# Smaug123/ray-tracing-fsharp

Measured on AMD Instinct MI355X. Metric: Mray/s (primary+secondary), higher is better.
Workload: dtype f64

## Files before the change

ray-tracing-fsharp_amd/csrc/rt_device.h:

```cpp
#pragma once
#include "rt_launch_consts.h"
#include <hip/hip_runtime.h>
#include <stdint.h>
#include <type_traits>

#include "rt_trig.h"

#pragma clang fp contract(off)

namespace rtd {

#define RTD_INLINE __device__ __forceinline__
#define RTD_AS3 __attribute__((address_space(3)))

typedef double d2 __attribute__((ext_vector_type(2)));
typedef int i2 __attribute__((ext_vector_type(2)));
typedef int i4 __attribute__((ext_vector_type(4)));

#define RTD_TOL 0.00000001
RTD_INLINE bool feq(double a, double b) { return fabs(a - b) < RTD_TOL; }
RTD_INLINE bool fpos(double a) { return a > RTD_TOL; }
enum { CMP_GT = 0, CMP_EQ = 1, CMP_LT = 2 };
RTD_INLINE int fcmp(double a, double b) {
    if (fabs(a - b) < RTD_TOL) return CMP_EQ;
// ... 16 lines not shown
    g = fma(g, r, g);
    h = fma(h, r, h);
    double e = fma(-g, g, x);
    g = fma(e, h, g);
    e = fma(-g, g, x);
    return fma(e, h, g);
}
RTD_INLINE double rcp_core(double s) {
    double r = __builtin_amdgcn_rcp(s);
    double e = fma(-s, r, 1.0);
    r = fma(r, e, r);
    e = fma(-s, r, 1.0);
    r = fma(r, e, r);
    e = fma(-s, r, 1.0);
    return fma(e, r, r);
}
RTD_INLINE double sqrt_above_tol(double x) {
    const double g = sqrt_core(x);
    return __builtin_isinf(x) ? x : g;
}
RTD_INLINE double inv_sqrt_above_tol(double x) {
    const double q = rcp_core(sqrt_core(x));
    return __builtin_isinf(x) ? 0.0 : q;
}
RTD_INLINE bool unitise(V3 v, V3 &out) {
    double d = dot(v, v);
    if (feq(d, 0.0)) return false;
    double factor = inv_sqrt_above_tol(d);
    out = vscale(factor, v);
    return true;
}

#ifdef RTD_STAGE_CLOCKS
#define RTD_CENSUS_WORDS 48
__device__ unsigned long long g_census[RTD_CENSUS_WORDS];
#define RTD_CENSUS_EVENT(i) atomicAdd(&g_census[i], 1ull)
#else
#define RTD_CENSUS_EVENT(i)
#endif

struct Rng { uint32_t x, y, z, w; };
RTD_INLINE uint32_t rng_next(Rng &r) {
    uint32_t t = r.x ^ (r.x << 11);
    r.x = r.y;
    r.y = r.z;
    r.z = r.w;
    r.w = r.w ^ (r.w >> 19) ^ (t ^ (t >> 8));
    return r.w;
}
RTD_INLINE double rng_get(Rng &r) {
    const double x = (double) __builtin_bswap32(rng_next(r));
    return fma(x, 0x1p-64 + 0x1p-96, x * 0x1p-32);
}

__host__ __device__ __forceinline__ uint64_t mix64(uint64_t z) {
    z ^= z >> 30;
    z *= 0xBF58476D1CE4E5B9ull;
    z ^= z >> 27;
    z *= 0x94D049BB133111EBull;
    z ^= z >> 31;
    return z;
}
#define RTD_GOLDEN 0x9E3779B97F4A7C15ull
RTD_INLINE uint32_t mod_m31(uint32_t x) {
    const uint32_t r = (x & 0x7FFFFFFFu) + (x >> 31);
    return r >= 2147483647u ? r - 2147483647u : r;
}
// ... 227 lines not shown
        "  v_min_f64 v[102:103], v[106:107], v[102:103]\n"
        "  s_waitcnt lgkmcnt(1)\n"
        "  v_add_f64 v[108:109], v[108:109], -%[oz]\n"
        "  v_mul_f64 v[108:109], %[iz], v[108:109]\n"
        "  v_max_f64 v[100:101], v[108:109], v[100:101]\n"
        "  v_add_f64 v[110:111], v[110:111], -%[oz]\n"
        "  v_mul_f64 v[110:111], %[iz], v[110:111]\n"
        "  v_cmp_lt_f64 vcc, 0, v[102:103]\n"
        "  v_min_f64 v[102:103], v[110:111], v[102:103]\n"
        "  v_cmp_ge_f64 %[save2], v[102:103], v[100:101]\n"
        "  s_and_b64 vcc, vcc, %[save2]\n"
        "  s_waitcnt lgkmcnt(0)\n"
        "  v_cndmask_b32 %[off], v113, v112, vcc\n"
        "  v_cndmask_b32 v113, 0, v115, vcc\n"
        "  v_alignbit_b32 %[pend], v114, %[pend], v113\n"
        "  s_mov_b64 exec, %[save]\n"
        "  s_branch 1b\n"
        "2:\n"
        : [off] "+v"(off), [pend] "+v"(pend), [ax] "=&v"(ax), [ay] "=&v"(ay), [az] "=&v"(az), [cnt] "=&s"(cnt), [save] "=&s"(save), [save2] "=&s"(save2)
        : [end] "s"(end), [stop] "s"(stop), [nx] "v"(c.nX), [ny] "v"(c.nY), [nz] "v"(c.nZ), [ox] "v"(o.x), [oy] "v"(o.y), [oz] "v"(o.z),
          [ix] "v"(c.ix), [iy] "v"(c.iy), [iz] "v"(c.iz), [inf] "s"(inf)
        : "vcc", "scc", "memory", "v100", "v101", "v102", "v103", "v104", "v105", "v106", "v107", "v108", "v109", "v110", "v111", "v112", "v113",
          "v114", "v115");
    return off;
}
#define RTD_PEND_MARK 0x4000u

struct WalkCtx32 {
    float ix, iy, iz;
    float cnx, cny, cnz;
    float cfx, cfy, cfz;
    int nX, nY, nZ;
};
RTD_INLINE void filter_axis(double o, double d, float bmax, float &inv, float &cn, float &cf, int &nOff) {
    inv = __builtin_amdgcn_rcpf((float) d);
    const float oi = (float) o * inv;
    const float m = fmaf(__builtin_fabsf(inv), bmax, __builtin_fabsf(oi)) * 0x1p-20f + 1e-30f;
    cn = -oi - m;
    cf = m - oi;
    nOff = (int) (((uint32_t) __double2hiint(d) >> 28) & 8u);
}
RTD_INLINE WalkCtx32 walk_ctx32(V3 o, V3 d, float bmax) {
    WalkCtx32 c;
    filter_axis(o.x, d.x, bmax, c.ix, c.cnx, c.cfx, c.nX);
    filter_axis(o.y, d.y, bmax, c.iy, c.cny, c.cfy, c.nY);
    filter_axis(o.z, d.z, bmax, c.iz, c.cnz, c.cfz, c.nZ);
    return c;
}
RTD_INLINE bool bbox_filter(const WalkCtx32 &c, float lox, float hix, float loy, float hiy, float loz, float hiz) {
    const float tn = __builtin_fmaxf(__builtin_fmaxf(__builtin_fmaxf(fmaf(c.nX ? hix : lox, c.ix, c.cnx), fmaf(c.nY ? hiy : loy, c.iy, c.cny)),
                                                     fmaf(c.nZ ? hiz : loz, c.iz, c.cnz)), 0.0f);
    const float tf = __builtin_fminf(__builtin_fminf(fmaf(c.nX ? lox : hix, c.ix, c.cfx), fmaf(c.nY ? loy : hiy, c.iy, c.cfy)), fmaf(c.nZ ? loz : hiz, c.iz, c.cfz));
    return !(tf < tn);
}
#ifdef RTD_STAGE_CLOCKS
#define RTD_TRIP_COUNT(S) S
#define RTD_TRIP_ARGS , unsigned &trips, unsigned &lanes
#define RTD_TRIP_OPS , [trips] "+s"(trips), [lanes] "+s"(lanes)
#else
#define RTD_TRIP_COUNT(S)
#define RTD_TRIP_ARGS
#define RTD_TRIP_OPS
#endif
RTD_INLINE int node_loop_lds32(int off, uint32_t &pend, int end, int stop, const WalkCtx32 &c RTD_TRIP_ARGS) {
    int ax, ay, az, cnt;
    unsigned long long save, save2;
#ifdef RTD_PK_FMA
    auto pk = [](float lo, float hi) { return ((unsigned long long) __float_as_uint(hi) << 32) | (unsigned long long) __float_as_uint(lo); };
    const unsigned long long pix = pk(c.ix, c.ix), piy = pk(c.iy, c.iy), piz = pk(c.iz, c.iz);
    const unsigned long long pcx = pk(c.cnx, c.cfx), pcy = pk(c.cny, c.cfy), pcz = pk(c.cnz, c.cfz);
#endif
    asm volatile(
        "s_waitcnt lgkmcnt(0)\n"
        "1:\n"
        "  v_cmp_gt_i32 vcc, %[end], %[off]\n"
        "  v_cmp_eq_u16 %[save2], 0, %[pend]\n"
        "  s_and_b64 vcc, vcc, %[save2]\n"
        "  s_bcnt1_i32_b64 %[cnt], vcc\n"
        "  s_cmp_le_u32 %[cnt], %[stop]\n"
        "  s_cbranch_scc1 2f\n"
        "  s_and_saveexec_b64 %[save], vcc\n"
        RTD_TRIP_COUNT("  s_add_u32 %[trips], %[trips], 1\n  s_add_u32 %[lanes], %[lanes], %[cnt]\n")
        "  v_add_u32 %[ax], %[off], %[nx]\n"
        "  v_add_u32 %[ay], %[off], %[ny]\n"
        "  v_add_u32 %[az], %[off], %[nz]\n"
        "  ds_read_b64 v[100:101], %[ax]\n"
        "  ds_read_b64 v[102:103], %[ay] offset:16\n"
        "  ds_read_b64 v[104:105], %[az] offset:32\n"
        "  ds_read_b128 v[106:109], %[off] offset:48\n"
        "  s_waitcnt lgkmcnt(3)\n"
#ifdef RTD_PK_FMA
        "  v_pk_fma_f32 v[100:101], v[100:101], %[pix], %[pcx] op_sel_hi:[1,0,1]\n"
        "  s_waitcnt lgkmcnt(2)\n"
        "  v_pk_fma_f32 v[102:103], v[102:103], %[piy], %[pcy] op_sel_hi:[1,0,1]\n"
        "  s_waitcnt lgkmcnt(1)\n"
        "  v_pk_fma_f32 v[104:105], v[104:105], %[piz], %[pcz] op_sel_hi:[1,0,1]\n"
#else
        "  v_fma_f32 v100, v100, %[ix], %[cnx]\n"
        "  v_fma_f32 v101, v101, %[ix], %[cfx]\n"
        "  s_waitcnt lgkmcnt(2)\n"
        "  v_fma_f32 v102, v102, %[iy], %[cny]\n"
        "  v_fma_f32 v103, v103, %[iy], %[cfy]\n"
        "  s_waitcnt lgkmcnt(1)\n"
        "  v_fma_f32 v104, v104, %[iz], %[cnz]\n"
        "  v_fma_f32 v105, v105, %[iz], %[cfz]\n"
#endif
        "  v_max3_f32 v100, v100, v102, v104\n"
        "  v_min3_f32 v101, v101, v103, v105\n"
        "  v_max_f32 v100, 0, v100\n"
        "  v_cmp_nlt_f32 vcc, v101, v100\n"
        "  s_waitcnt lgkmcnt(0)\n"
        "  v_cndmask_b32 %[off], v107, v106, vcc\n"
        "  v_cndmask_b32 v107, 0, v109, vcc\n"
        "  v_alignbit_b32 %[pend], v108, %[pend], v107\n"
        "  s_mov_b64 exec, %[save]\n"
        "  s_branch 1b\n"
        "2:\n"
        : [off] "+v"(off), [pend] "+v"(pend), [ax] "=&v"(ax), [ay] "=&v"(ay), [az] "=&v"(az), [cnt] "=&s"(cnt), [save] "=&s"(save), [save2] "=&s"(save2) RTD_TRIP_OPS
        : [end] "s"(end), [stop] "s"(stop), [nx] "v"(c.nX), [ny] "v"(c.nY), [nz] "v"(c.nZ), [ix] "v"(c.ix), [iy] "v"(c.iy), [iz] "v"(c.iz),
          [cnx] "v"(c.cnx), [cny] "v"(c.cny), [cnz] "v"(c.cnz), [cfx] "v"(c.cfx), [cfy] "v"(c.cfy), [cfz] "v"(c.cfz)
#ifdef RTD_PK_FMA
          , [pix] "v"(pix), [piy] "v"(piy), [piz] "v"(piz), [pcx] "v"(pcx), [pcy] "v"(pcy), [pcz] "v"(pcz)
#endif
        : "vcc", "scc", "memory", "v100", "v101", "v102", "v103", "v104", "v105", "v106", "v107", "v108", "v109");
    return off;
}
RTD_INLINE int pend_pop(uint32_t &pend) {
    const uint32_t lo = pend & 0xFFFFu;
    const uint32_t e = lo != 0u ? lo : (pend >> 16);
    pend = lo != 0u ? (pend & 0xFFFF0000u) : 0u;
    return (int) (e & (RTD_PEND_MARK - 1u));
}
template <bool LDS>
RTD_INLINE void leaf_test(const SceneView<LDS> &sc, V3 o, V3 d, WalkCtx &c, Walk &w) {
    typedef typename Ptrs<LDS>::bp bp;
    bp rec = node_at<LDS>(sc, w.off & (RTD_LEAF - 1));
    const int next = *(typename Ptrs<LDS>::ip) (rec + 100), prim = *(typename Ptrs<LDS>::ip) (rec + 104);
    const d2 g0 = sc.geo[prim * 3 + 0], g1 = sc.geo[prim * 3 + 1];
    const double t = sphere_first_intersection(o, d, mk(g0.x, g0.y, g1.x), g1.y);
    const double a = t * t;
    if (a < c.bestF || (a == c.bestF && prim < w.best)) { c.bestF = a; w.best = prim; w.bestLen = t; }
    w.off = next;
// ... 16 lines not shown
        "  v_cmp_eq_u32 %[save2], 0, %[pend1]\n"
        "  s_and_b64 vcc, vcc, %[save2]\n"
        "  s_bcnt1_i32_b64 %[cnt], vcc\n"
        "  s_cmp_le_u32 %[cnt], %[stop]\n"
        "  s_cbranch_scc1 2f\n"
        "  s_and_saveexec_b64 %[save], vcc\n"
        "  v_add_u32 %[ax], %[off], %[nx]\n"
        "  v_add_u32 %[ay], %[off], %[ny]\n"
        "  v_add_u32 %[az], %[off], %[nz]\n"
        "  v_cmp_gt_i32 vcc, %[lim], %[off]\n"
        "  s_bcnt1_i32_b64 %[cnt], vcc\n"
        "  s_cmp_ge_u32 %[cnt], %[thr]\n"
        "  s_cbranch_scc1 3f\n"
        "  s_and_saveexec_b64 %[save2], vcc\n"
        "  ds_read_b64 v[100:101], %[ax]\n"
        "  ds_read_b64 v[102:103], %[ay] offset:16\n"
        "  ds_read_b64 v[104:105], %[az] offset:32\n"
        "  ds_read_b128 v[106:109], %[off] offset:48\n"
        "  s_andn2_b64 exec, %[save2], exec\n"
        "  global_load_dwordx2 v[100:101], %[ax], %[base]\n"
        "  global_load_dwordx2 v[102:103], %[ay], %[base] offset:16\n"
        "  global_load_dwordx2 v[104:105], %[az], %[base] offset:32\n"
        "  global_load_dwordx4 v[106:109], %[off], %[base] offset:48\n"
        "  s_mov_b64 exec, %[save2]\n"
        "  s_branch 4f\n"
        "3:\n"
        "  s_mov_b64 exec, vcc\n"
        "  ds_read_b64 v[100:101], %[ax]\n"
        "  ds_read_b64 v[102:103], %[ay] offset:16\n"
        "  ds_read_b64 v[104:105], %[az] offset:32\n"
        "  ds_read_b128 v[106:109], %[off] offset:48\n"
        "4:\n"
        "  s_waitcnt vmcnt(0) lgkmcnt(0)\n"
        "  v_fma_f32 v100, v100, %[ix], %[cnx]\n"
        "  v_fma_f32 v101, v101, %[ix], %[cfx]\n"
        "  v_fma_f32 v102, v102, %[iy], %[cny]\n"
        "  v_fma_f32 v103, v103, %[iy], %[cfy]\n"
        "  v_fma_f32 v104, v104, %[iz], %[cnz]\n"
        "  v_fma_f32 v105, v105, %[iz], %[cfz]\n"
        "  v_max3_f32 v100, v100, v102, v104\n"
        "  v_min3_f32 v101, v101, v103, v105\n"
        "  v_max_f32 v100, 0, v100\n"
        "  v_cmp_nlt_f32 vcc, v101, v100\n"
        "  v_cndmask_b32 %[off], v107, v106, vcc\n"
        "  v_cndmask_b32 v108, 0, v108, vcc\n"
        "  v_cmp_ne_u32 %[save3], 0, v108\n"
        "  v_cmp_eq_u32 vcc, 0, %[pend0]\n"
        "  s_and_b64 vcc, %[save3], vcc\n"
        "  v_cndmask_b32 %[pend0], %[pend0], v108, vcc\n"
        "  s_andn2_b64 vcc, %[save3], vcc\n"
        "  v_cndmask_b32 %[pend1], %[pend1], v108, vcc\n"
        "  s_mov_b64 exec, %[save]\n"
        "  s_branch 1b\n"
        "2:\n"
        : [off] "+v"(off), [pend0] "+v"(pend0), [pend1] "+v"(pend1), [ax] "=&v"(ax), [ay] "=&v"(ay), [az] "=&v"(az), [cnt] "=&s"(cnt), [save] "=&s"(save),
          [save2] "=&s"(save2), [save3] "=&s"(save3)
        : [end] "s"(end), [lim] "s"(lim), [thr] "s"(thr), [stop] "s"(stop), [base] "s"(base), [nx] "v"(c.nX), [ny] "v"(c.nY), [nz] "v"(c.nZ), [ix] "v"(c.ix), [iy] "v"(c.iy), [iz] "v"(c.iz),
          [cnx] "v"(c.cnx), [cny] "v"(c.cny), [cnz] "v"(c.cnz), [cfx] "v"(c.cfx), [cfy] "v"(c.cfy), [cfz] "v"(c.cfz)
        : "vcc", "scc", "memory", "v100", "v101", "v102", "v103", "v104", "v105", "v106", "v107", "v108", "v109");
    return off;
}
RTD_INLINE int node_loop_hyb16(int off, uint32_t &pend, const unsigned char *base, int lim, int thr, int end, int stop, const WalkCtx32 &c RTD_TRIP_ARGS) {
    int ax, ay, az, cnt;
    unsigned long long save, save2;
#define RTD_HYB_TAIL                                                                                                                  \
        "  v_max3_f32 v100, v100, v102, v104\n"                                                                                       \
        "  v_min3_f32 v101, v101, v103, v105\n"                                                                                       \
        "  v_max_f32 v100, 0, v100\n"                                                                                                 \
        "  v_cmp_nlt_f32 vcc, v101, v100\n"                                                                                           \
        "  s_waitcnt vmcnt(0) lgkmcnt(0)\n"                                                                                           \
        "  v_cndmask_b32 %[off], v107, v106, vcc\n"                                                                                   \
        "  v_cndmask_b32 v107, 0, v109, vcc\n"                                                                                        \
        "  v_alignbit_b32 %[pend], v108, %[pend], v107\n"                                                                             \
        "  s_mov_b64 exec, %[save]\n"                                                                                                 \
        "  s_branch 1b\n"
    asm volatile(
        "s_waitcnt vmcnt(0) lgkmcnt(0)\n"
        "1:\n"
        "  v_cmp_gt_i32 vcc, %[end], %[off]\n"
        "  v_cmp_eq_u16 %[save2], 0, %[pend]\n"
        "  s_and_b64 vcc, vcc, %[save2]\n"
        "  s_bcnt1_i32_b64 %[cnt], vcc\n"
        "  s_cmp_le_u32 %[cnt], %[stop]\n"
        "  s_cbranch_scc1 2f\n"
        "  s_and_saveexec_b64 %[save], vcc\n"
        RTD_TRIP_COUNT("  s_add_u32 %[trips], %[trips], 1\n")
        "  v_cmp_gt_i32 vcc, %[lim], %[off]\n"
        "  v_add_u32 %[ax], %[off], %[nx]\n"
        "  v_add_u32 %[ay], %[off], %[ny]\n"
        "  v_add_u32 %[az], %[off], %[nz]\n"
        "  s_bcnt1_i32_b64 %[cnt], vcc\n"
        "  s_cmp_ge_u32 %[cnt], %[thr]\n"
        "  s_cbranch_scc1 3f\n"
        "  s_and_saveexec_b64 %[save2], vcc\n"
        "  ds_read_b64 v[100:101], %[ax]\n"
        "  ds_read_b64 v[102:103], %[ay] offset:16\n"
        "  ds_read_b64 v[104:105], %[az] offset:32\n"
        "  ds_read_b128 v[106:109], %[off] offset:48\n"
        "  s_andn2_b64 exec, %[save2], exec\n"
        "  global_load_dwordx2 v[100:101], %[ax], %[base]\n"
        "  global_load_dwordx2 v[102:103], %[ay], %[base] offset:16\n"
        "  global_load_dwordx2 v[104:105], %[az], %[base] offset:32\n"
        "  global_load_dwordx4 v[106:109], %[off], %[base] offset:48\n"
        "  s_mov_b64 exec, %[save2]\n"
        RTD_TRIP_COUNT("  s_bcnt1_i32_b64 %[cnt], %[save2]\n  s_add_u32 %[lanes], %[lanes], %[cnt]\n")
        "  s_waitcnt vmcnt(0) lgkmcnt(0)\n"
        "  v_fma_f32 v100, v100, %[ix], %[cnx]\n"
        "  v_fma_f32 v101, v101, %[ix], %[cfx]\n"
        "  v_fma_f32 v102, v102, %[iy], %[cny]\n"
        "  v_fma_f32 v103, v103, %[iy], %[cfy]\n"
        "  v_fma_f32 v104, v104, %[iz], %[cnz]\n"
        "  v_fma_f32 v105, v105, %[iz], %[cfz]\n"
        RTD_HYB_TAIL
        "3:\n"
        RTD_TRIP_COUNT("  s_add_u32 %[lanes], %[lanes], %[cnt]\n")
        "  s_mov_b64 exec, vcc\n"
        "  ds_read_b64 v[100:101], %[ax]\n"
        "  ds_read_b64 v[102:103], %[ay] offset:16\n"
        "  ds_read_b64 v[104:105], %[az] offset:32\n"
        "  ds_read_b128 v[106:109], %[off] offset:48\n"
        "  s_waitcnt lgkmcnt(3)\n"
        "  v_fma_f32 v100, v100, %[ix], %[cnx]\n"
        "  v_fma_f32 v101, v101, %[ix], %[cfx]\n"
        "  s_waitcnt lgkmcnt(2)\n"
        "  v_fma_f32 v102, v102, %[iy], %[cny]\n"
        "  v_fma_f32 v103, v103, %[iy], %[cfy]\n"
        "  s_waitcnt lgkmcnt(1)\n"
        "  v_fma_f32 v104, v104, %[iz], %[cnz]\n"
        "  v_fma_f32 v105, v105, %[iz], %[cfz]\n"
        RTD_HYB_TAIL
        "2:\n"
        : [off] "+v"(off), [pend] "+v"(pend), [ax] "=&v"(ax), [ay] "=&v"(ay), [az] "=&v"(az), [cnt] "=&s"(cnt), [save] "=&s"(save), [save2] "=&s"(save2) RTD_TRIP_OPS
        : [end] "s"(end), [lim] "s"(lim), [thr] "s"(thr), [stop] "s"(stop), [base] "s"(base), [nx] "v"(c.nX), [ny] "v"(c.nY), [nz] "v"(c.nZ), [ix] "v"(c.ix), [iy] "v"(c.iy), [iz] "v"(c.iz),
          [cnx] "v"(c.cnx), [cny] "v"(c.cny), [cnz] "v"(c.cnz), [cfx] "v"(c.cfx), [cfy] "v"(c.cfy), [cfz] "v"(c.cfz)
        : "vcc", "scc", "memory", "v100", "v101", "v102", "v103", "v104", "v105", "v106", "v107", "v108", "v109");
#undef RTD_HYB_TAIL
    return off;
}
RTD_INLINE int pend_pop_wide(uint32_t &pend0, uint32_t &pend1) {
    const uint32_t e = pend0;
    pend0 = pend1;
    pend1 = 0u;
    return (int) ((e & RTD_PEND_WIDE) ? (e & ~RTD_PEND_WIDE) : (e & (RTD_PEND_MARK - 1u)));
}

#define RTD_IMPLIED_DD 1.0e6
template <bool LDS>
RTD_INLINE void leaf_test_object_exact(const SceneView<LDS> &sc, V3 o, V3 d, double &bestF, Walk &w, int prim, bool implied) {
    const d2 g0 = sc.geo[prim * 3 + 0], g1 = sc.geo[prim * 3 + 1];
    const V3 diff = vsub(o, mk(g0.x, g0.y, g1.x));
    const double b = dot(d, diff);
    const double dd = dot(diff, diff);
    const double cc = dd - g1.y;
    const double disc = (b * b - cc);
    const bool eq = fzero(disc), gt = fgreater0(disc);
// ... 400 lines not shown
```

ray-tracing-fsharp_amd/csrc/rt_render_kernel.h:

```cpp
#pragma once
#include "rt_device.h"

namespace rtd {

struct RenderParams {
    const CameraParams *cam_ptr;
    int32_t depth;
    int32_t spp;
    int32_t max_w, max_h;
    SceneOffsets off;
    const unsigned char *scene_image;
    const TexRec *tex;
    const uint8_t *texels;
    uint64_t seed_key;
    int32_t cols;
    int32_t row_first, row_stride;
    int32_t n_rows;
    int32_t k;
    int32_t chunk;
    int32_t leaf_wait;
    int32_t yield_lanes;
    int32_t refill_lanes;
    int32_t park;
    int32_t park_l;
// ... 63 lines not shown
}
template <> RTD_INLINE SceneView<false> make_view<false, true>(const RenderParams &p, const unsigned char *) {
    SceneView<false> v;
    const unsigned char *b = p.scene_image;
    v.node = b + p.off.node32;
    v.geo = (const d2 *) (b + p.off.geo);
    v.meta = (const i2 *) (b + p.off.meta);
    v.mat = (const double *) (b + p.off.mat);
    v.n_nodes = p.off.n_nodes; v.n_bounded = p.off.n_bounded; v.n_unbounded = p.off.n_unbounded;
    v.first = 0; v.end = v.n_nodes * RTD_NODE32_BYTES;
    v.tex = p.tex; v.texels = p.texels; v.lds_lim = 0; v.lds_thr = 65; v.narrow = (v.n_bounded + v.n_unbounded) < 16384 ? 1 : 0;
    return v;
}
template <> RTD_INLINE SceneView<false> make_view<false, false>(const RenderParams &p, const unsigned char *) {
    SceneView<false> v;
    const unsigned char *b = p.scene_image;
    v.node = b + p.off.node;
    v.geo = (const d2 *) (b + p.off.geo);
    v.meta = (const i2 *) (b + p.off.meta);
    v.mat = (const double *) (b + p.off.mat);
    v.n_nodes = p.off.n_nodes; v.n_bounded = p.off.n_bounded; v.n_unbounded = p.off.n_unbounded;
    v.first = 0; v.end = v.n_nodes * RTD_NODE_BYTES;
    v.tex = p.tex; v.texels = p.texels; v.lds_lim = 0; v.lds_thr = 65; v.narrow = (v.n_bounded + v.n_unbounded) < 16384 ? 1 : 0;
    return v;
}

struct StageStats {
    uint32_t refill, trips, leaf, shade, refillLanes, shadeLanes, slow, slowLanes, parkedLanes;
    unsigned long long tRefill, tSlow, tWalk, tShade;
    unsigned long long loopTrips, loopLanes;
    unsigned long long tLoop, tLeaf, tUnb, tCam, tLamb;
#ifdef RTD_STAGE_CLOCKS
    uint32_t turns, lambBatches, lambLanes, newRefills, newItems, unparkL, unparkA, storeBlocksL, storeLanesL, storeBlocksA,
        lightBatches, lightLanes, missLanes, ranges, flushes, leafLanes, unparkBatchesL, unparkBatchesA, slowLanesByStyle[8], slowBatchesByStyle[8];
#endif
};
#ifdef RTD_STAGE_CLOCKS
#define RTD_CENSUS(S) S
#else
#define RTD_CENSUS(S)
#endif

#ifdef RTD_STAGE_CLOCKS
#define RTD_CLK true
#else
#define RTD_CLK false
#endif

enum { L_IDLE = 0, L_WALK = 1, L_DONE = 2, L_SLOW = 3, L_LAMB = 4, L_TEX = 5 };

template <bool LDS, bool COUNT, bool TEX, bool LOG>
struct Sched {
    const RenderParams &p;
    const SceneView<LDS> &sc;
    Counters &cnt;
    StageStats &ss;
    unsigned char *pool;
    RTD_AS3 unsigned char *poolLds;
    uint32_t parked;
    uint32_t parkedL;
    uint32_t parkedT;
    const int end;
    int st;
    V3 o, d;
    Walk w;
    Rng rng;
    uint32_t colour, slotOff;
// ... 151 lines not shown
            after_reflection(reflection<LDS, false>(sc, w.best, strike, o, d, colour, rng, TEX ? texc : RTD_NO_TEX));
        }
    }

    RTD_INLINE void stage_tex() {
        if (!TEX) return;
        if (__builtin_amdgcn_ballot_w64(st == L_TEX) == 0ull) return;
        if (st == L_TEX) {
            const V3 strike = walk(o, d, w.bestLen);
            texc = texture_colour_at_inline(sc.tex, sc.texels, textured(sc.meta[w.best]), strike, nullptr);
            st = L_SLOW;
        }
    }

    RTD_INLINE void stage_lamb() {
        if (__builtin_amdgcn_ballot_w64(st == L_LAMB) == 0ull) return;
        RTD_CENSUS(ss.lambBatches++; ss.lambLanes += (uint32_t) __popcll(__builtin_amdgcn_ballot_w64(st == L_LAMB));)
        const unsigned long long k0 = RTD_CLK ? __builtin_amdgcn_s_memtime() : 0ull;
        if (st == L_LAMB) {
            const bool inside = bounces < 0;
            bounces &= 0x7FFFFFFF;
            lambert_bounce<LDS>(sc, w.best, sc.meta[w.best], o, inside, o, d, colour, rng);
            after_reflection(false);
        }
        if (RTD_CLK) ss.tLamb += __builtin_amdgcn_s_memtime() - k0;
    }

    RTD_INLINE void stage_walk() {
        const unsigned long long walkM0 = __builtin_amdgcn_ballot_w64(st == L_WALK);
        if (walkM0 == 0ull) return;
        const int nBusy = __popcll(__builtin_amdgcn_ballot_w64(st != L_IDLE));
        const int stop = (nBusy - p.leaf_wait) > 0 ? (nBusy - p.leaf_wait) : 0;
        if constexpr (!COUNT) {
            const WalkCtx32 f = walk_ctx32(o, d, p.off.bmax);
            double bestF = (w.best < 0) ? __builtin_inf() : w.bestLen * w.bestLen;
            const bool implied = p.off.box_implied != 0;
            if (RTD_CLK) ss.trips++;
            unsigned long long walkM = walkM0, doneM = __builtin_amdgcn_ballot_w64(st == L_DONE);
            for (;;) {
                const unsigned long long k0 = RTD_CLK ? __builtin_amdgcn_s_memtime() : 0ull;
#ifdef RTD_STAGE_CLOCKS
                unsigned nTrips = 0u, nLanes = 0u;
#define RTD_TRIP_PASS , nTrips, nLanes
#else
#define RTD_TRIP_PASS
#endif
                if constexpr (LDS) w.off = node_loop_lds32(w.off, pend, end, stop, f RTD_TRIP_PASS);
                else if (sc.narrow) w.off = node_loop_hyb16(w.off, pend, (const unsigned char *) sc.node, sc.lds_lim, sc.lds_thr, end, stop, f RTD_TRIP_PASS);
                else w.off = node_loop_glb32(w.off, pend, pend1, (const unsigned char *) sc.node, sc.lds_lim, sc.lds_thr, end, stop, f);
#ifdef RTD_STAGE_CLOCKS
                ss.loopTrips += nTrips; ss.loopLanes += nLanes;
#endif
#undef RTD_TRIP_PASS
                const unsigned long long k1 = RTD_CLK ? __builtin_amdgcn_s_memtime() : 0ull;
                if (RTD_CLK && __builtin_amdgcn_ballot_w64(pend != 0u) != 0ull) ss.leaf++;
                RTD_CENSUS(ss.leafLanes += (uint32_t) __popcll(__builtin_amdgcn_ballot_w64(pend != 0u));)
                if (pend != 0u) {
                    int prim;
                    if (LDS || sc.narrow) {
                        prim = pend_pop(pend);
                        if (pend == 0u) { pend = pend1; pend1 = 0u; }
                    } else prim = pend_pop_wide(pend, pend1);
                    leaf_test_object_exact<LDS>(sc, o, d, bestF, w, prim, implied);
                }
                if (RTD_CLK) { ss.tLoop += k1 - k0; ss.tLeaf += __builtin_amdgcn_s_memtime() - k1; }
                const bool fin = (st == L_WALK) && (w.off >= end) && pend == 0u;
                if (fin) st = L_DONE;
                const unsigned long long finM = walkM & __builtin_amdgcn_ballot_w64(w.off >= end) & __builtin_amdgcn_ballot_w64(pend == 0u);
                walkM &= ~finM; doneM |= finM;
                if (walkM == 0ull || __popcll(doneM) >= p.yield_lanes) break;
            }
            return;
        }
        WalkCtx c = walk_ctx(d, w);
        for (;;) {
            for (;;) {
                const bool act = w.off < end;
                const int nAct = __popcll(__builtin_amdgcn_ballot_w64(act));
                if (nAct <= stop) break;
                if (COUNT) ss.trips++;
                if (act) {
                    if (COUNT) cnt.aabb++;
// ... 439 lines not shown
    const int lane = threadIdx.x & 63;
    const int wave = __builtin_amdgcn_readfirstlane((int) (threadIdx.x >> 6));

    const uint32_t ldsNodes = (!LDS && !COUNT) ? stage_nodes32<BLOCK>(p, smem) : 0u;
    const uint32_t sceneBytes = LDS ? stage_scene<BLOCK, !COUNT>(p, smem) : (uint32_t) ((!LDS && !COUNT) ? p.lds_node_bytes : 0);
    SceneView<LDS> scv = make_view<LDS, !COUNT>(p, smem);
    scv.lds_lim = (int) ldsNodes;
    scv.lds_thr = p.lds_node_thr;
    const SceneView<LDS> &sc = scv;
    const uint32_t P = (uint32_t) p.chunk;
    RTD_AS3 uint32_t *wv = (RTD_AS3 uint32_t *) (smem + sceneBytes) + (size_t) wave * (MODE >= 4 ? 0u : MODE == 1 ? RTD_WAVE_WORDS_A(P) : RTD_WAVE_WORDS(P));
    RTD_AS3 uint32_t *acc = wv;
    RTD_AS3 uint32_t *pix = wv + 6u * P;
    RTD_AS3 uint32_t *live = pix + 4u * P;
    RTD_AS3 uint32_t *cand = live + P;
    unsigned char *pool = p.park_pool + ((size_t) blockIdx.x * (BLOCK / 64) + (size_t) wave) * (size_t) RTD_PARK_ENTRY_BYTES *
                                        (size_t) (p.park + (p.park_l_lds ? 0 : p.park_l) + (TEX ? p.park : 0));
    RTD_AS3 unsigned char *poolLds = (RTD_AS3 unsigned char *) (smem + sceneBytes) + (size_t) (BLOCK / 64) * (MODE >= 4 ? 0u : MODE == 1 ? RTD_WAVE_WORDS_A(P) : RTD_WAVE_WORDS(P)) * 4u +
                                     (size_t) wave * (size_t) RTD_PARK_L_LDS_BYTES * (size_t) p.park_l;

    const uint64_t nLocal = (uint64_t) p.n_rows * (uint64_t) p.cols;
    const uint32_t k = (uint32_t) p.k;
    const uint32_t n1 = 2u * k + 1u;
    const int n2s = p.spp - 2 * p.k - 1;
    const uint32_t n2 = n2s > 0 ? (uint32_t) n2s : 0u;

    const unsigned long long tStart = COUNT ? __builtin_amdgcn_s_memrealtime() : 0ull;
    Counters cnt; cnt.rays = cnt.aabb = cnt.prim = cnt.refl = 0;
    StageStats ss; ss.refill = ss.trips = ss.leaf = ss.shade = ss.refillLanes = ss.shadeLanes = ss.slow = ss.slowLanes = ss.parkedLanes = 0;
    ss.tRefill = ss.tSlow = ss.tWalk = ss.tShade = 0ull;
    ss.tLoop = ss.tLeaf = ss.tUnb = ss.tCam = ss.tLamb = 0ull;
    ss.loopTrips = ss.loopLanes = 0ull;
#ifdef RTD_STAGE_CLOCKS
    ss.turns = ss.lambBatches = ss.lambLanes = ss.newRefills = ss.newItems = ss.unparkL = ss.unparkA = ss.storeBlocksL = ss.storeLanesL = ss.storeBlocksA = 0u;
    ss.lightBatches = ss.lightLanes = ss.missLanes = ss.ranges = ss.flushes = ss.leafLanes = ss.unparkBatchesL = ss.unparkBatchesA = 0u;
    for (int i = 0; i < 8; ++i) ss.slowLanesByStyle[i] = ss.slowBatchesByStyle[i] = 0u;
#endif
    uint32_t earlyCount = 0;
    uint64_t sampleCount = 0;

    if constexpr (MODE >= 4) run_rays<LDS, COUNT, TEX, MODE == 5>(p, sc, pool, poolLds, cnt, ss);
    else if (MODE == 2) run_stream<LDS, COUNT, TEX>(p, sc, pool, poolLds, wv, n1, n2, cnt, ss, sampleCount);
    else
    for (;;) {
        uint32_t unit = 0;
        if (lane == 0) unit = atomicAdd(p.queue, 1u);
        unit = __builtin_amdgcn_readfirstlane(unit);
        const unsigned long long first = (unsigned long long) unit * P;
        if (first >= nLocal) break;
        const uint32_t npx = (uint32_t) ((nLocal - first < (unsigned long long) P) ? (nLocal - first) : (unsigned long long) P);

        for (uint32_t i = (uint32_t) lane; i < 6u * P; i += 64u) acc[i] = 0u;
        if (MODE == 1 && (uint32_t) lane < P) acc[10u * P + lane] = 0u;
        unsigned long long lp = 0;
        if ((uint32_t) lane < npx) {
            lp = first + (uint32_t) lane;
            uint32_t lr = (uint32_t) (lp / (unsigned long long) p.cols);
            uint32_t c = (uint32_t) (lp - (unsigned long long) lr * (unsigned long long) p.cols);
            uint32_t r = (uint32_t) p.row_first + lr * (uint32_t) p.row_stride;
            uint64_t pkey = pixel_key(p.seed_key, (uint64_t) r * (uint64_t) p.cols + c);
            pix[lane * 4 + 0] = (uint32_t) (p.max_h - (int) r - 1);
            pix[lane * 4 + 1] = (uint32_t) ((int) c - p.max_w);
            pix[lane * 4 + 2] = (uint32_t) pkey;
            pix[lane * 4 + 3] = (uint32_t) (pkey >> 32);
            const CameraParams *cp = p.cam_ptr;
            asm volatile("" : "+s"(cp));
            uint32_t c2;
// ... 72 lines not shown
            atomicMax(&p.counters[7], 0x4000000000000000ull - tStart);
        }
    }
    if ((COUNT || RTD_CLK) && lane == 0) {
        atomicAdd(&p.counters[8], (unsigned long long) ss.refill);
        atomicAdd(&p.counters[9], (unsigned long long) ss.trips);
        atomicAdd(&p.counters[10], (unsigned long long) ss.leaf);
        atomicAdd(&p.counters[11], (unsigned long long) ss.shade);
        atomicAdd(&p.counters[12], (unsigned long long) ss.refillLanes);
        atomicAdd(&p.counters[13], (unsigned long long) ss.shadeLanes);
        atomicAdd(&p.counters[20], (unsigned long long) ss.slow);
        atomicAdd(&p.counters[21], (unsigned long long) ss.slowLanes);
        atomicAdd(&p.counters[22], (unsigned long long) ss.parkedLanes);
        atomicAdd(&p.counters[23], ss.tRefill);
        atomicAdd(&p.counters[24], ss.tSlow);
        atomicAdd(&p.counters[25], ss.tWalk);
        atomicAdd(&p.counters[26], ss.tShade);
        if (RTD_CLK) {
            atomicAdd(&p.counters[27], ss.tLoop);
            atomicAdd(&p.counters[28], ss.tLeaf);
            atomicAdd(&p.counters[29], ss.tUnb);
            atomicAdd(&p.counters[30], ss.tCam);
            atomicAdd(&p.counters[31], ss.tLamb);
            if (!COUNT) { atomicAdd(&p.counters[14], ss.loopTrips); atomicAdd(&p.counters[15], ss.loopLanes); }
#ifdef RTD_STAGE_CLOCKS
            if (!COUNT && MODE == 2) {
                const uint32_t cz[16] = {ss.turns, ss.lambBatches, ss.lambLanes, ss.newRefills, ss.newItems, ss.unparkL, ss.unparkA, ss.storeBlocksL, ss.storeLanesL,
                                         ss.storeBlocksA, ss.lightBatches, ss.lightLanes, ss.missLanes, ss.ranges, ss.flushes, ss.leafLanes};
                for (int i = 0; i < 16; ++i) atomicAdd(&g_census[i], (unsigned long long) cz[i]);
                for (int i = 0; i < 8; ++i) { atomicAdd(&g_census[16 + i], (unsigned long long) ss.slowLanesByStyle[i]); atomicAdd(&g_census[24 + i], (unsigned long long) ss.slowBatchesByStyle[i]); }
                const unsigned long long sz[12] = {ss.refill, ss.trips, ss.leaf, ss.shade, ss.refillLanes, ss.shadeLanes, ss.slow, ss.slowLanes, ss.loopTrips, ss.loopLanes,
                                                   ss.unparkBatchesL, ss.unparkBatchesA};
                for (int i = 0; i < 12; ++i) atomicAdd(&g_census[36 + i], sz[i]);
            }
#endif
        }
    }
    if (lane == 0) {
        atomicAdd(&p.counters[4], (unsigned long long) s);
        atomicAdd(&p.counters[5], (unsigned long long) e);
    }
}


RTD_INLINE uint32_t cost_bucket(unsigned long long pair, uint32_t n1) {
    const uint32_t cost = (uint32_t) (pair >> 32);
    const uint32_t b = (cost * 4u) / n1;
    return b >= RTD_COST_BUCKETS ? RTD_COST_BUCKETS - 1u : b;
}
RTD_INLINE void sort_slice(unsigned int n, unsigned int &lo, unsigned int &hi) {
    const unsigned int per = (n + gridDim.x - 1u) / gridDim.x;
    lo = blockIdx.x * per;
    hi = lo + per < n ? lo + per : n;
    if (lo > n) lo = n;
}
__global__ void sort_hist_kernel(const unsigned long long *pairs, const unsigned int *count, uint32_t n1, unsigned int *hist) {
    __shared__ unsigned int local[RTD_COST_BUCKETS];
    if (threadIdx.x < RTD_COST_BUCKETS) local[threadIdx.x] = 0u;
    __syncthreads();
    unsigned int lo, hi;
    sort_slice(*count, lo, hi);
    for (unsigned int i = lo + threadIdx.x; i < hi; i += blockDim.x) atomicAdd(&local[cost_bucket(pairs[i], n1)], 1u);
    __syncthreads();
    if (threadIdx.x < RTD_COST_BUCKETS && local[threadIdx.x] != 0u) atomicAdd(&hist[threadIdx.x], local[threadIdx.x]);
}
__global__ void sort_offsets_kernel(const unsigned int *hist, unsigned int *offsets) {
// ... 29 lines not shown
```

ray-tracing-fsharp_amd/csrc/rtfs_amd.hip:

```cpp
#include "../../include/rtfs_amd.h"
#include "rt_device.h"
#include "rt_launch_plan.h"
#include "rt_render_kernel.h"
#include "rt_scene.h"

#include <hip/hip_runtime.h>

#include <dlfcn.h>

#include <atomic>
#include <chrono>
#include <cstddef>
#include <cstdio>
#include <map>
#include <memory>
#include <mutex>
#include <new>
#include <set>
#include <string>
#include <system_error>
#include <tuple>
#include <utility>
#include <vector>

// ... 1375 lines not shown
__global__ void __launch_bounds__(1024) k_pixel_candidates(const RenderParams p, const CameraParams cam, int n, const int32_t *rowcol, uint32_t *out) {
    extern __shared__ __attribute__((aligned(16))) unsigned char smem[];
    (void) stage_scene<1024, true>(p, smem);
    const SceneView<true> sc = make_view<true, true>(p, smem);
    const int i = blockIdx.x * 1024 + threadIdx.x;
    if (i >= n) return;
    uint32_t second = 0u;
    const uint32_t first = pixel_candidates<true, true>(sc, cam, rowcol[i * 2], rowcol[i * 2 + 1], second);
    out[i * 2] = first;
    out[i * 2 + 1] = second;
}
__global__ void k_pixel_candidates_glb(const RenderParams p, const CameraParams cam, int n, const int32_t *rowcol, uint32_t *out) {
    const SceneView<false> sc = make_view<false, true>(p, nullptr);
    const int i = blockIdx.x * blockDim.x + threadIdx.x;
    if (i >= n) return;
    uint32_t second = 0u;
    const uint32_t first = pixel_candidates<false, true>(sc, cam, rowcol[i * 2], rowcol[i * 2 + 1], second);
    out[i * 2] = first;
    out[i * 2 + 1] = second;
}
__global__ void k_bbox_filter(int n, const double *rays, const double *boxes, const float *boxes32, float bmax, int32_t *out) {
    int i = blockIdx.x * blockDim.x + threadIdx.x;
    if (i >= n) return;
    const double *r = rays + i * 6, *b = boxes + i * 6;
    const float *f = boxes32 + i * 6;
    d2 bx, by, bz;
    bx.x = b[0]; bx.y = b[3]; by.x = b[1]; by.y = b[4]; bz.x = b[2]; bz.y = b[5];
    const V3 o = mk(r[0], r[1], r[2]), d = mk(r[3], r[4], r[5]);
    const bool exact = bbox_hits(1.0 / d.x, 1.0 / d.y, 1.0 / d.z, o, bx, by, bz);
    const WalkCtx32 c = walk_ctx32(o, d, bmax);
    const float nx = c.nX ? f[3] : f[0], fx = c.nX ? f[0] : f[3], ny = c.nY ? f[4] : f[1], fy = c.nY ? f[1] : f[4], nz = c.nZ ? f[5] : f[2], fz = c.nZ ? f[2] : f[5];
    float t0 = nx, t1 = fx, t2 = ny, t3 = fy, t4 = nz, t5 = fz;
    unsigned long long m;
    asm volatile("v_fma_f32 %0, %0, %7, %10\n\tv_fma_f32 %1, %1, %7, %13\n\t"
                 "v_fma_f32 %2, %2, %8, %11\n\tv_fma_f32 %3, %3, %8, %14\n\t"
                 "v_fma_f32 %4, %4, %9, %12\n\tv_fma_f32 %5, %5, %9, %15\n\t"
                 "v_max3_f32 %0, %0, %2, %4\n\tv_min3_f32 %1, %1, %3, %5\n\tv_max_f32 %0, 0, %0\n\tv_cmp_nlt_f32_e64 %6, %1, %0"
                 : "+v"(t0), "+v"(t1), "+v"(t2), "+v"(t3), "+v"(t4), "+v"(t5), "=s"(m)
                 : "v"(c.ix), "v"(c.iy), "v"(c.iz), "v"(c.cnx), "v"(c.cny), "v"(c.cnz), "v"(c.cfx), "v"(c.cfy), "v"(c.cfz));
    const bool filter = (m >> (threadIdx.x & 63)) & 1ull;
    out[i] = (exact ? 1 : 0) | (filter ? 2 : 0) | (bbox_filter(c, f[0], f[3], f[1], f[4], f[2], f[5]) ? 4 : 0);
}
__global__ void k_trace_ray(const RenderParams p, int depth, int n, const double *rays, uint32_t *rng, uint8_t *col_out) {
    int i = blockIdx.x * blockDim.x + threadIdx.x;
    if (i >= n) return;
    const SceneView<false> sc = make_view<false>(p, nullptr);
    const double *r = rays + i * 6;
    Rng g; g.x = rng[i * 4]; g.y = rng[i * 4 + 1]; g.z = rng[i * 4 + 2]; g.w = rng[i * 4 + 3];
    Counters cnt; cnt.rays = cnt.aabb = cnt.prim = cnt.refl = 0;
    uint32_t c = trace_ray<false, false>(sc, depth, mk(r[0], r[1], r[2]), mk(r[3], r[4], r[5]), g, cnt);
    st_rgb(col_out + i * 3, c);
    rng[i * 4] = g.x; rng[i * 4 + 1] = g.y; rng[i * 4 + 2] = g.z; rng[i * 4 + 3] = g.w;
}
__global__ void k_texture(const RenderParams p, int tex, int n, const double *pts, double *uv, uint8_t *col) {
    int i = blockIdx.x * blockDim.x + threadIdx.x;
    if (i >= n) return;
    double u[2] = {__builtin_nan(""), __builtin_nan("")};
    uint32_t c = texture_colour_at(p.tex, p.texels, tex, mk(pts[i * 3], pts[i * 3 + 1], pts[i * 3 + 2]), u);
    if (uv) { uv[i * 2] = u[0]; uv[i * 2 + 1] = u[1]; }
    st_rgb(col + i * 3, c);
}

template <class K, class... A> static void launch_n(K kernel, int n, A... args) {
    if (n) hipLaunchKernelGGL(kernel, dim3((unsigned) ((n + 255) / 256)), dim3(256), 0, 0, args...);
}

template <class F> static int hook(const char *entry, int32_t device, F &&body) {
    return guarded(entry, [&]() -> int {
        DeviceGuard guard;
        const int rc = guard.enter(device);
// ... 252 lines not shown
```

Measured before the change: 33800.

## Rescale walk context so clamp modifier replaces max, and build it lazily

The float walk context now scales the inverse direction by a power-of-two sigma chosen from the scene bound. Entry distances then fit in [0,1], so the FMA's clamp modifier can replace the separate v_max with zero in every node-loop variant. The context is also built only when enough lanes will actually enter the node loop, using inline-asm conversions to control scheduling. This removes one ALU op per node test and skips context setup on turns where the loop would not run. In exchange it adds ballot checks, and the X-axis near value is clamped to at most 1, which narrows the filter and relies on the scaling bounding t.

Measured after the change: 33900 (median of 6 runs). Within noise of the previous version (+0.3%).

```diff
diff --git a/ray-tracing-fsharp_amd/csrc/rt_device.h b/ray-tracing-fsharp_amd/csrc/rt_device.h
--- a/ray-tracing-fsharp_amd/csrc/rt_device.h
+++ b/ray-tracing-fsharp_amd/csrc/rt_device.h
@@ -72,7 +72,7 @@
 }
 
 #ifdef RTD_STAGE_CLOCKS
-#define RTD_CENSUS_WORDS 48
+#define RTD_CENSUS_WORDS 49
 __device__ unsigned long long g_census[RTD_CENSUS_WORDS];
 #define RTD_CENSUS_EVENT(i) atomicAdd(&g_census[i], 1ull)
 #else
@@ -366,24 +366,55 @@
     float cfx, cfy, cfz;
     int nX, nY, nZ;
 };
-RTD_INLINE void filter_axis(double o, double d, float bmax, float &inv, float &cn, float &cf, int &nOff) {
-    inv = __builtin_amdgcn_rcpf((float) d);
-    const float oi = (float) o * inv;
-    const float m = fmaf(__builtin_fabsf(inv), bmax, __builtin_fabsf(oi)) * 0x1p-20f + 1e-30f;
+RTD_INLINE int filter_sigma_exp(float bmax) {
+    const uint32_t u = __float_as_uint(bmax);
+    const int e = (int) ((u >> 23) & 0xFFu) - 125 + ((u & 0x7FFFFFu) != 0u ? 1 : 0);
+    return e < 0 ? 0 : (e > 20 ? 20 : e);
+}
+RTD_INLINE float filter_sigma(int e) { return __uint_as_float((uint32_t) (127 - e) << 23); }
+RTD_INLINE float filter_guard(int e) { return __uint_as_float(__float_as_uint(1e-30f) - ((uint32_t) e << 23)); }
+RTD_INLINE void filter_axis32(float o, float d, uint32_t dSign, float bmax, int e, float &inv, float &cn, float &cf, int &nOff) {
+    inv = __builtin_amdgcn_rcpf(d) * filter_sigma(e);
+    const float oi = o * inv;
+    const float m = fmaf(__builtin_fabsf(inv), bmax, __builtin_fabsf(oi)) * 0x1p-20f + filter_guard(e);
     cn = -oi - m;
     cf = m - oi;
-    nOff = (int) (((uint32_t) __double2hiint(d) >> 28) & 8u);
+    nOff = (int) (dSign >> 28);
+}
+RTD_INLINE void filter_axis(double o, double d, float bmax, int e, float &inv, float &cn, float &cf, int &nOff) {
+    filter_axis32((float) o, (float) d, (uint32_t) __double2hiint(d) & 0x80000000u, bmax, e, inv, cn, cf, nOff);
 }
 RTD_INLINE WalkCtx32 walk_ctx32(V3 o, V3 d, float bmax) {
     WalkCtx32 c;
-    filter_axis(o.x, d.x, bmax, c.ix, c.cnx, c.cfx, c.nX);
-    filter_axis(o.y, d.y, bmax, c.iy, c.cny, c.cfy, c.nY);
-    filter_axis(o.z, d.z, bmax, c.iz, c.cnz, c.cfz, c.nZ);
+    const int e = filter_sigma_exp(bmax);
+    filter_axis(o.x, d.x, bmax, e, c.ix, c.cnx, c.cfx, c.nX);
+    filter_axis(o.y, d.y, bmax, e, c.iy, c.cny, c.cfy, c.nY);
+    filter_axis(o.z, d.z, bmax, e, c.iz, c.cnz, c.cfz, c.nZ);
     return c;
 }
+RTD_INLINE void filter_axis_here(double o, double d, float bmax, int e, const float *after, float &inv, float &cn, float &cf, int &nOff) {
+    float o32, d32;
+    uint32_t dSign;
+    if (after) asm volatile("v_cvt_f32_f64 %0, %1" : "=v"(o32) : "v"(o), "v"(after[0]), "v"(after[1]));
+    else asm volatile("v_cvt_f32_f64 %0, %1" : "=v"(o32) : "v"(o));
+    asm volatile("v_cvt_f32_f64 %0, %1" : "=v"(d32) : "v"(d));
+    asm volatile("v_and_b32 %0, 0x80000000, %1" : "=v"(dSign) : "v"(__double2hiint(d)));
+    filter_axis32(o32, d32, dSign, bmax, e, inv, cn, cf, nOff);
+}
+RTD_INLINE WalkCtx32 walk_ctx32_here(V3 o, V3 d, float bmax) {
+    WalkCtx32 c;
+    asm volatile("" : "+s"(bmax));
+    const int e = filter_sigma_exp(bmax);
+    filter_axis_here(o.x, d.x, bmax, e, nullptr, c.ix, c.cnx, c.cfx, c.nX);
+    const float doneX[2] = {c.cnx, c.cfx};
+    filter_axis_here(o.y, d.y, bmax, e, doneX, c.iy, c.cny, c.cfy, c.nY);
+    const float doneY[2] = {c.cny, c.cfy};
+    filter_axis_here(o.z, d.z, bmax, e, doneY, c.iz, c.cnz, c.cfz, c.nZ);
+    return c;
+}
 RTD_INLINE bool bbox_filter(const WalkCtx32 &c, float lox, float hix, float loy, float hiy, float loz, float hiz) {
-    const float tn = __builtin_fmaxf(__builtin_fmaxf(__builtin_fmaxf(fmaf(c.nX ? hix : lox, c.ix, c.cnx), fmaf(c.nY ? hiy : loy, c.iy, c.cny)),
-                                                     fmaf(c.nZ ? hiz : loz, c.iz, c.cnz)), 0.0f);
+    const float tx = __builtin_fminf(__builtin_fmaxf(fmaf(c.nX ? hix : lox, c.ix, c.cnx), 0.0f), 1.0f);
+    const float tn = __builtin_fmaxf(__builtin_fmaxf(tx, fmaf(c.nY ? hiy : loy, c.iy, c.cny)), fmaf(c.nZ ? hiz : loz, c.iz, c.cnz));
     const float tf = __builtin_fminf(__builtin_fminf(fmaf(c.nX ? lox : hix, c.ix, c.cfx), fmaf(c.nY ? loy : hiy, c.iy, c.cfy)), fmaf(c.nZ ? loz : hiz, c.iz, c.cfz));
     return !(tf < tn);
 }
@@ -429,8 +460,9 @@
         "  v_pk_fma_f32 v[102:103], v[102:103], %[piy], %[pcy] op_sel_hi:[1,0,1]\n"
         "  s_waitcnt lgkmcnt(1)\n"
         "  v_pk_fma_f32 v[104:105], v[104:105], %[piz], %[pcz] op_sel_hi:[1,0,1]\n"
+        "  v_max_f32 v100, v100, v100 clamp\n"
 #else
-        "  v_fma_f32 v100, v100, %[ix], %[cnx]\n"
+        "  v_fma_f32 v100, v100, %[ix], %[cnx] clamp\n"
         "  v_fma_f32 v101, v101, %[ix], %[cfx]\n"
         "  s_waitcnt lgkmcnt(2)\n"
         "  v_fma_f32 v102, v102, %[iy], %[cny]\n"
@@ -441,7 +473,6 @@
 #endif
         "  v_max3_f32 v100, v100, v102, v104\n"
         "  v_min3_f32 v101, v101, v103, v105\n"
-        "  v_max_f32 v100, 0, v100\n"
         "  v_cmp_nlt_f32 vcc, v101, v100\n"
         "  s_waitcnt lgkmcnt(0)\n"
         "  v_cndmask_b32 %[off], v107, v106, vcc\n"
@@ -524,7 +555,7 @@
         "  ds_read_b128 v[106:109], %[off] offset:48\n"
         "4:\n"
         "  s_waitcnt vmcnt(0) lgkmcnt(0)\n"
-        "  v_fma_f32 v100, v100, %[ix], %[cnx]\n"
+        "  v_fma_f32 v100, v100, %[ix], %[cnx] clamp\n"
         "  v_fma_f32 v101, v101, %[ix], %[cfx]\n"
         "  v_fma_f32 v102, v102, %[iy], %[cny]\n"
         "  v_fma_f32 v103, v103, %[iy], %[cfy]\n"
@@ -532,7 +563,6 @@
         "  v_fma_f32 v105, v105, %[iz], %[cfz]\n"
         "  v_max3_f32 v100, v100, v102, v104\n"
         "  v_min3_f32 v101, v101, v103, v105\n"
-        "  v_max_f32 v100, 0, v100\n"
         "  v_cmp_nlt_f32 vcc, v101, v100\n"
         "  v_cndmask_b32 %[off], v107, v106, vcc\n"
         "  v_cndmask_b32 v108, 0, v108, vcc\n"
@@ -558,7 +588,6 @@
 #define RTD_HYB_TAIL                                                                                                                  \
         "  v_max3_f32 v100, v100, v102, v104\n"                                                                                       \
         "  v_min3_f32 v101, v101, v103, v105\n"                                                                                       \
-        "  v_max_f32 v100, 0, v100\n"                                                                                                 \
         "  v_cmp_nlt_f32 vcc, v101, v100\n"                                                                                           \
         "  s_waitcnt vmcnt(0) lgkmcnt(0)\n"                                                                                           \
         "  v_cndmask_b32 %[off], v107, v106, vcc\n"                                                                                   \
@@ -597,7 +626,7 @@
         "  s_mov_b64 exec, %[save2]\n"
         RTD_TRIP_COUNT("  s_bcnt1_i32_b64 %[cnt], %[save2]\n  s_add_u32 %[lanes], %[lanes], %[cnt]\n")
         "  s_waitcnt vmcnt(0) lgkmcnt(0)\n"
-        "  v_fma_f32 v100, v100, %[ix], %[cnx]\n"
+        "  v_fma_f32 v100, v100, %[ix], %[cnx] clamp\n"
         "  v_fma_f32 v101, v101, %[ix], %[cfx]\n"
         "  v_fma_f32 v102, v102, %[iy], %[cny]\n"
         "  v_fma_f32 v103, v103, %[iy], %[cfy]\n"
@@ -612,7 +641,7 @@
         "  ds_read_b64 v[104:105], %[az] offset:32\n"
         "  ds_read_b128 v[106:109], %[off] offset:48\n"
         "  s_waitcnt lgkmcnt(3)\n"
-        "  v_fma_f32 v100, v100, %[ix], %[cnx]\n"
+        "  v_fma_f32 v100, v100, %[ix], %[cnx] clamp\n"
         "  v_fma_f32 v101, v101, %[ix], %[cfx]\n"
         "  s_waitcnt lgkmcnt(2)\n"
         "  v_fma_f32 v102, v102, %[iy], %[cny]\n"
diff --git a/ray-tracing-fsharp_amd/csrc/rt_render_kernel.h b/ray-tracing-fsharp_amd/csrc/rt_render_kernel.h
--- a/ray-tracing-fsharp_amd/csrc/rt_render_kernel.h
+++ b/ray-tracing-fsharp_amd/csrc/rt_render_kernel.h
@@ -119,7 +119,8 @@
     unsigned long long tLoop, tLeaf, tUnb, tCam, tLamb;
 #ifdef RTD_STAGE_CLOCKS
     uint32_t turns, lambBatches, lambLanes, newRefills, newItems, unparkL, unparkA, storeBlocksL, storeLanesL, storeBlocksA,
-        lightBatches, lightLanes, missLanes, ranges, flushes, leafLanes, unparkBatchesL, unparkBatchesA, slowLanesByStyle[8], slowBatchesByStyle[8];
+        lightBatches, lightLanes, missLanes, ranges, flushes, leafLanes, unparkBatchesL, unparkBatchesA, slowLanesByStyle[8], slowBatchesByStyle[8],
+        ctxBuilds;
 #endif
 };
 #ifdef RTD_STAGE_CLOCKS
@@ -337,7 +338,8 @@
         const int nBusy = __popcll(__builtin_amdgcn_ballot_w64(st != L_IDLE));
         const int stop = (nBusy - p.leaf_wait) > 0 ? (nBusy - p.leaf_wait) : 0;
         if constexpr (!COUNT) {
-            const WalkCtx32 f = walk_ctx32(o, d, p.off.bmax);
+            WalkCtx32 f;
+            bool haveCtx = false;
             double bestF = (w.best < 0) ? __builtin_inf() : w.bestLen * w.bestLen;
             const bool implied = p.off.box_implied != 0;
             if (RTD_CLK) ss.trips++;
@@ -350,9 +352,19 @@
 #else
 #define RTD_TRIP_PASS
 #endif
-                if constexpr (LDS) w.off = node_loop_lds32(w.off, pend, end, stop, f RTD_TRIP_PASS);
-                else if (sc.narrow) w.off = node_loop_hyb16(w.off, pend, (const unsigned char *) sc.node, sc.lds_lim, sc.lds_thr, end, stop, f RTD_TRIP_PASS);
-                else w.off = node_loop_glb32(w.off, pend, pend1, (const unsigned char *) sc.node, sc.lds_lim, sc.lds_thr, end, stop, f);
+                if (!haveCtx) {
+                    const bool room = (LDS || sc.narrow) ? (pend & 0xFFFFu) == 0u : pend1 == 0u;
+                    if (__popcll(__builtin_amdgcn_ballot_w64(w.off < end) & __builtin_amdgcn_ballot_w64(room)) > stop) {
+                        f = walk_ctx32_here(o, d, p.off.bmax);
+                        haveCtx = true;
+                        RTD_CENSUS(ss.ctxBuilds++;)
+                    }
+                }
+                if (haveCtx) {
+                    if constexpr (LDS) w.off = node_loop_lds32(w.off, pend, end, stop, f RTD_TRIP_PASS);
+                    else if (sc.narrow) w.off = node_loop_hyb16(w.off, pend, (const unsigned char *) sc.node, sc.lds_lim, sc.lds_thr, end, stop, f RTD_TRIP_PASS);
+                    else w.off = node_loop_glb32(w.off, pend, pend1, (const unsigned char *) sc.node, sc.lds_lim, sc.lds_thr, end, stop, f);
+                }
 #ifdef RTD_STAGE_CLOCKS
                 ss.loopTrips += nTrips; ss.loopLanes += nLanes;
 #endif
@@ -858,7 +870,7 @@
     ss.tLoop = ss.tLeaf = ss.tUnb = ss.tCam = ss.tLamb = 0ull;
     ss.loopTrips = ss.loopLanes = 0ull;
 #ifdef RTD_STAGE_CLOCKS
-    ss.turns = ss.lambBatches = ss.lambLanes = ss.newRefills = ss.newItems = ss.unparkL = ss.unparkA = ss.storeBlocksL = ss.storeLanesL = ss.storeBlocksA = 0u;
+    ss.ctxBuilds = ss.turns = ss.lambBatches = ss.lambLanes = ss.newRefills = ss.newItems = ss.unparkL = ss.unparkA = ss.storeBlocksL = ss.storeLanesL = ss.storeBlocksA = 0u;
     ss.lightBatches = ss.lightLanes = ss.missLanes = ss.ranges = ss.flushes = ss.leafLanes = ss.unparkBatchesL = ss.unparkBatchesA = 0u;
     for (int i = 0; i < 8; ++i) ss.slowLanesByStyle[i] = ss.slowBatchesByStyle[i] = 0u;
 #endif
@@ -997,6 +1009,7 @@
                 const unsigned long long sz[12] = {ss.refill, ss.trips, ss.leaf, ss.shade, ss.refillLanes, ss.shadeLanes, ss.slow, ss.slowLanes, ss.loopTrips, ss.loopLanes,
                                                    ss.unparkBatchesL, ss.unparkBatchesA};
                 for (int i = 0; i < 12; ++i) atomicAdd(&g_census[36 + i], sz[i]);
+                atomicAdd(&g_census[48], (unsigned long long) ss.ctxBuilds);
             }
 #endif
         }
diff --git a/ray-tracing-fsharp_amd/csrc/rtfs_amd.hip b/ray-tracing-fsharp_amd/csrc/rtfs_amd.hip
--- a/ray-tracing-fsharp_amd/csrc/rtfs_amd.hip
+++ b/ray-tracing-fsharp_amd/csrc/rtfs_amd.hip
@@ -1431,10 +1431,10 @@
     const float nx = c.nX ? f[3] : f[0], fx = c.nX ? f[0] : f[3], ny = c.nY ? f[4] : f[1], fy = c.nY ? f[1] : f[4], nz = c.nZ ? f[5] : f[2], fz = c.nZ ? f[2] : f[5];
     float t0 = nx, t1 = fx, t2 = ny, t3 = fy, t4 = nz, t5 = fz;
     unsigned long long m;
-    asm volatile("v_fma_f32 %0, %0, %7, %10\n\tv_fma_f32 %1, %1, %7, %13\n\t"
+    asm volatile("v_fma_f32 %0, %0, %7, %10 clamp\n\tv_fma_f32 %1, %1, %7, %13\n\t"
                  "v_fma_f32 %2, %2, %8, %11\n\tv_fma_f32 %3, %3, %8, %14\n\t"
                  "v_fma_f32 %4, %4, %9, %12\n\tv_fma_f32 %5, %5, %9, %15\n\t"
-                 "v_max3_f32 %0, %0, %2, %4\n\tv_min3_f32 %1, %1, %3, %5\n\tv_max_f32 %0, 0, %0\n\tv_cmp_nlt_f32_e64 %6, %1, %0"
+                 "v_max3_f32 %0, %0, %2, %4\n\tv_min3_f32 %1, %1, %3, %5\n\tv_cmp_nlt_f32_e64 %6, %1, %0"
                  : "+v"(t0), "+v"(t1), "+v"(t2), "+v"(t3), "+v"(t4), "+v"(t5), "=s"(m)
                  : "v"(c.ix), "v"(c.iy), "v"(c.iz), "v"(c.cnx), "v"(c.cny), "v"(c.cnz), "v"(c.cfx), "v"(c.cfy), "v"(c.cfz));
     const bool filter = (m >> (threadIdx.x & 63)) & 1ull;
```
